# umautobots/LONER

Measured on AMD Instinct MI355X. Metric: training rays/sec, higher is better.
Workload: dtype f32

## Files before the change

### loner_amd/csrc/lnr_density_bf3.hip

```cpp
#include "lnr_f16_common.h"

typedef __bf16 bf16x8 __attribute__((ext_vector_type(8)));
typedef __bf16 bf16x2 __attribute__((ext_vector_type(2)));

#define BF3_TS 36
#ifndef LNR_BF3_FWD_OCC
#define LNR_BF3_FWD_OCC 3
#endif

struct Frag3 { u32x4 t[3]; };

__device__ __forceinline__ void bf3_split_pair(float x, float y, uint32_t& p0, uint32_t& p1, uint32_t& p2) {
    p0 = __builtin_bit_cast(uint32_t, bf16x2{(__bf16)x, (__bf16)y});
    asm volatile("" : "+v"(p0));
    float rx = x - __uint_as_float(p0 << 16), ry = y - __uint_as_float(p0 & 0xFFFF0000u);
    p1 = __builtin_bit_cast(uint32_t, bf16x2{(__bf16)rx, (__bf16)ry});
    asm volatile("" : "+v"(p1));
    rx -= __uint_as_float(p1 << 16);
    ry -= __uint_as_float(p1 & 0xFFFF0000u);
    p2 = __builtin_bit_cast(uint32_t, bf16x2{(__bf16)rx, (__bf16)ry});
}
__device__ __forceinline__ void bf3_split8(const float v[8], Frag3& f) {
#pragma unroll
    for (int q = 0; q < 4; ++q) {
        uint32_t p0, p1, p2;
        bf3_split_pair(v[2 * q], v[2 * q + 1], p0, p1, p2);
        f.t[0][q] = p0; f.t[1][q] = p1; f.t[2][q] = p2;
    }
}
#define BF3_M(a, b, acc) __builtin_amdgcn_mfma_f32_16x16x32_bf16(__builtin_bit_cast(bf16x8, a), __builtin_bit_cast(bf16x8, b), acc, 0, 0, 0)
#define BF3_FOR_TERMS(X) X(0, 2) X(2, 0) X(1, 1) X(0, 1) X(1, 0) X(0, 0)
__device__ __forceinline__ f32x4 bf3_mfma6(const Frag3& a, const Frag3& b, f32x4 acc) {
    acc = BF3_M(a.t[0], b.t[2], acc);
    acc = BF3_M(a.t[2], b.t[0], acc);
    acc = BF3_M(a.t[1], b.t[1], acc);
    acc = BF3_M(a.t[0], b.t[1], acc);
    acc = BF3_M(a.t[1], b.t[0], acc);
    acc = BF3_M(a.t[0], b.t[0], acc);
    return acc;
}

__device__ __forceinline__ void bf3_load_x2(const float* __restrict__ fb, uint32_t plane_bytes, uint32_t m_even, float x[2][8]) {
#pragma unroll
    for (int i = 0; i < 8; ++i) {
        const float2 v = ld32<float2>(fb, (uint32_t)i * plane_bytes + m_even * 4u);
        x[0][i] = v.x; x[1][i] = v.y;
    }
}

template <int HT>
__global__ void __launch_bounds__(LNR_DENSITY_BLOCK, LNR_BF3_FWD_OCC)
mlp_forward_bf3_kernel(const float* __restrict__ params, const float* __restrict__ feat, int64_t m_pad, int64_t n_points,
                       const int32_t* __restrict__ n_rays_dev, int n_rays, int n_samples, float* __restrict__ sigma, int32_t* __restrict__ clip_flag) {
    constexpr int H = 16 * HT;
    const int lane = threadIdx.x & 63, wave = threadIdx.x >> 6, nw = blockDim.x >> 6;
    const int c = lane & 15, g = lane >> 4;
    Frag3 wa[HT]; float wo[HT][4];
#pragma unroll
    for (int jt = 0; jt < HT; ++jt) {
        float v[8];
#pragma unroll
        for (int i = 0; i < 8; ++i) v[i] = params[(16 * jt + c) * 32 + 8 * g + i];
        bf3_split8(v, wa[jt]);
#pragma unroll
        for (int r = 0; r < 4; ++r) wo[jt][r] = params[H * 32 + 16 * jt + 4 * g + r];
    }
    const int64_t M = live_samples(n_points, n_rays_dev, n_rays, n_samples);
    const int64_t n_tiles = M > 0 ? (M + 31) / 32 : 0;
    const int64_t stride = (int64_t)gridDim.x * nw;
    int64_t tile = (int64_t)blockIdx.x * nw + wave;
    if (tile >= n_tiles) return;
    const float* fb = feat + (size_t)(8 * g) * m_pad;
    const uint32_t plane_bytes = (uint32_t)m_pad * 4u;
    float cur[2][8], nxt[2][8];
    bf3_load_x2(fb, plane_bytes, (uint32_t)(tile * 32 + 2 * c), cur);
    bf3_load_x2(fb, plane_bytes, (uint32_t)((tile + stride < n_tiles ? tile + stride : tile) * 32 + 2 * c), nxt);
    while (tile < n_tiles) {
        const int64_t nt = tile + stride, nt2 = nt + stride;
        float nx2[2][8];
        bf3_load_x2(fb, plane_bytes, (uint32_t)((nt2 < n_tiles ? nt2 : tile) * 32 + 2 * c), nx2);
        __builtin_amdgcn_sched_barrier(0);
        Frag3 xb0, xb1;
        bf3_split8(cur[0], xb0);
        bf3_split8(cur[1], xb1);
        f32x4 Z0[HT], Z1[HT];
#pragma unroll
        for (int jt = 0; jt < HT; ++jt) { Z0[jt] = f32x4{0.0f, 0.0f, 0.0f, 0.0f}; Z1[jt] = f32x4{0.0f, 0.0f, 0.0f, 0.0f}; }
#define BF3_X(IA, IB)                                                                          \
    _Pragma("unroll") for (int jt = 0; jt < HT; ++jt) { Z0[jt] = BF3_M(wa[jt].t[IA], xb0.t[IB], Z0[jt]); Z1[jt] = BF3_M(wa[jt].t[IA], xb1.t[IB], Z1[jt]); }
        BF3_FOR_TERMS(BF3_X)
#undef BF3_X
        float p0 = 0.0f, p1 = 0.0f;
#pragma unroll
        for (int jt = 0; jt < HT; ++jt)
#pragma unroll
            for (int r = 0; r < 4; ++r) { p0 += wo[jt][r] * fmaxf(Z0[jt][r], 0.0f); p1 += wo[jt][r] * fmaxf(Z1[jt][r], 0.0f); }
        p0 += __shfl_xor(p0, 16, 64); p1 += __shfl_xor(p1, 16, 64);
        p0 += __shfl_xor(p0, 32, 64); p1 += __shfl_xor(p1, 32, 64);
        const int64_t m = tile * 32 + 2 * c;
        if (g == 0 && m < M) {
            p0 = finite_or_clipped<false>(p0, clip_flag);
            if (m + 1 < M) { p1 = finite_or_clipped<false>(p1, clip_flag); *reinterpret_cast<float2*>(sigma + m) = make_float2(p0, p1); }
            else sigma[m] = p0;
        }
#pragma unroll
        for (int t = 0; t < 2; ++t)
#pragma unroll
            for (int i = 0; i < 8; ++i) { cur[t][i] = nxt[t][i]; nxt[t][i] = nx2[t][i]; }
        tile = nt;
    }
}

template <int HT>
struct Bf3Lds {
    static constexpr int H = 16 * HT, KB = (HT + 1) / 2, NW = LNR_DENSITY_BLOCK / 64;
    static constexpr size_t N_MLP = (size_t)H * 32 + 16 * H;
    static constexpr size_t OFF_T = N_MLP * sizeof(float);
    static constexpr size_t OFF_WA = OFF_T + (size_t)NW * H * BF3_TS * sizeof(float);
    static constexpr size_t OFF_WT = OFF_WA + (size_t)3 * HT * 64 * 16;
    static constexpr size_t BYTES = OFF_WT + (size_t)3 * 2 * KB * 64 * 16;
};

template <int HT>
__global__ void __launch_bounds__(LNR_DENSITY_BLOCK, 2)
mlp_backward_bf3_kernel(const float* __restrict__ params, int n_mlp, const float* __restrict__ feat, int64_t m_pad, int64_t n_points,
                        const int32_t* __restrict__ n_rays_dev, int n_rays, int n_samples, const float* __restrict__ d_sigma,
                        float* __restrict__ dfeat, float* __restrict__ slabs, int want_dfeat) {
    extern __shared__ __attribute__((aligned(16))) float smem[];
    using L = Bf3Lds<HT>;
    constexpr int H = 16 * HT, KB = L::KB;
    const int nw = blockDim.x >> 6;
    const int lane = threadIdx.x & 63, wave = threadIdx.x >> 6;
    const int c = lane & 15, g = lane >> 4;
    float* dW = smem;
    float* T = reinterpret_cast<float*>(reinterpret_cast<char*>(smem) + L::OFF_T) + wave * (H * BF3_TS);
    u32x4* WA = reinterpret_cast<u32x4*>(reinterpret_cast<char*>(smem) + L::OFF_WA);
    u32x4* WT = reinterpret_cast<u32x4*>(reinterpret_cast<char*>(smem) + L::OFF_WT);
    for (int i = threadIdx.x; i < n_mlp; i += blockDim.x) dW[i] = 0.0f;
    for (int job = wave; job < HT + 2 * KB; job += nw) {
        float v[8];
        if (job < HT) {
#pragma unroll
            for (int i = 0; i < 8; ++i) v[i] = params[(16 * job + c) * 32 + 8 * g + i];
        } else {
            const int it = (job - HT) / KB, kb = (job - HT) % KB;
#pragma unroll
            for (int i = 0; i < 8; ++i) {
                const int n = 32 * kb + (i < 4 ? 4 * g + i : 16 + 4 * g + (i - 4));
                v[i] = n < H ? params[n * 32 + 16 * it + c] : 0.0f;
            }
        }
        Frag3 f;
        bf3_split8(v, f);
#pragma unroll
        for (int t3 = 0; t3 < 3; ++t3) {
            if (job < HT) WA[(t3 * HT + job) * 64 + lane] = f.t[t3];
            else WT[(t3 * 2 * KB + (job - HT)) * 64 + lane] = f.t[t3];
        }
    }
    float wo[HT][4];
#pragma unroll
    for (int jt = 0; jt < HT; ++jt)
#pragma unroll
        for (int r = 0; r < 4; ++r) wo[jt][r] = params[H * 32 + 16 * jt + 4 * g + r];
    __syncthreads();
    f32x4 dW1_acc[HT][2];
    float dWo_acc[HT][4];
#pragma unroll
    for (int jt = 0; jt < HT; ++jt) {
        dW1_acc[jt][0] = f32x4{0.0f, 0.0f, 0.0f, 0.0f};
        dW1_acc[jt][1] = f32x4{0.0f, 0.0f, 0.0f, 0.0f};
#pragma unroll
        for (int r = 0; r < 4; ++r) dWo_acc[jt][r] = 0.0f;
    }

    const int64_t M = live_samples(n_points, n_rays_dev, n_rays, n_samples);
    const int64_t n_tiles = M > 0 ? (M + 31) / 32 : 0;
    const int64_t stride = (int64_t)gridDim.x * nw;
    const uint32_t plane_bytes = (uint32_t)m_pad * 4u;
    const float* fb = feat + (size_t)(8 * g) * m_pad;
    const float* fc = feat + (size_t)c * m_pad;
    float* db = dfeat + (size_t)(4 * g) * m_pad;
    int64_t tile = (int64_t)blockIdx.x * nw + wave;
    float xcur[2][8], dcur[2];
    auto load_front = [&](int64_t tl, float (&x)[2][8], float (&ds)[2]) {
        const int64_t m = tl * 32 + 2 * c;
        bf3_load_x2(fb, plane_bytes, (uint32_t)m, x);
        const float v0 = d_sigma[m < M ? m : M - 1], v1 = d_sigma[m + 1 < M ? m + 1 : M - 1];
        ds[0] = m < M ? v0 : 0.0f;
        ds[1] = m + 1 < M ? v1 : 0.0f;
    };
    float xnxt[2][8], dnxt[2];
    if (tile < n_tiles) { load_front(tile, xcur, dcur); load_front(tile + stride < n_tiles ? tile + stride : tile, xnxt, dnxt); }
    while (tile < n_tiles) {
        const int64_t nt = tile + stride;
        const int64_t nt2 = nt + stride;
        float xnx2[2][8], dnx2[2];
        load_front(nt2 < n_tiles ? nt2 : tile, xnx2, dnx2);
        const bool any = (dcur[0] != 0.0f) | (dcur[1] != 0.0f);
        if (__ballot(any) == 0ull) {
            if (want_dfeat) {
#pragma unroll
                for (int k = 0; k < 8; ++k)
                    st32<float2>(db, (uint32_t)(16 * (k >> 2) + (k & 3)) * plane_bytes + (uint32_t)(tile * 32 + 2 * c) * 4u, make_float2(0.0f, 0.0f));
            }
        } else {
            float xraw[2][8];
#pragma unroll
            for (int it = 0; it < 2; ++it) {
                const uint32_t off = (uint32_t)(16 * it) * plane_bytes + (uint32_t)(tile * 32 + 8 * g) * 4u;
                const float4 a = ld32<float4>(fc, off), b = ld32<float4>(fc, off + 16u);
                xraw[it][0] = a.x; xraw[it][1] = a.y; xraw[it][2] = a.z; xraw[it][3] = a.w;
                xraw[it][4] = b.x; xraw[it][5] = b.y; xraw[it][6] = b.z; xraw[it][7] = b.w;
            }
            Frag3 xf[2];
            bf3_split8(xcur[0], xf[0]);
            bf3_split8(xcur[1], xf[1]);
            int wl = lane;
            asm volatile("" : "+v"(wl));
            float dz[HT][2][4];
#pragma unroll
            for (int jt = 0; jt < HT; ++jt) {
                Frag3 wa;
#pragma unroll
                for (int t3 = 0; t3 < 3; ++t3) wa.t[t3] = WA[(t3 * HT + jt) * 64 + wl];
                f32x4 Z0 = f32x4{0.0f, 0.0f, 0.0f, 0.0f}, Z1 = f32x4{0.0f, 0.0f, 0.0f, 0.0f};
#define BF3_X(IA, IB) Z0 = BF3_M(wa.t[IA], xf[0].t[IB], Z0); Z1 = BF3_M(wa.t[IA], xf[1].t[IB], Z1);
                BF3_FOR_TERMS(BF3_X)
#undef BF3_X
#pragma unroll
                for (int r = 0; r < 4; ++r) {
                    dWo_acc[jt][r] += dcur[0] * fmaxf(Z0[r], 0.0f) + dcur[1] * fmaxf(Z1[r], 0.0f);
                    dz[jt][0][r] = Z0[r] > 0.0f ? dcur[0] * wo[jt][r] : 0.0f;
                    dz[jt][1][r] = Z1[r] > 0.0f ? dcur[1] * wo[jt][r] : 0.0f;
                    *reinterpret_cast<float2*>(T + (16 * jt + 4 * g + r) * BF3_TS + 2 * c) = make_float2(dz[jt][0][r], dz[jt][1][r]);
                }
            }
            Frag3 xs[2];
            bf3_split8(xraw[0], xs[0]);
            bf3_split8(xraw[1], xs[1]);
#pragma unroll
            for (int it = 0; it < 2; ++it)
#pragma unroll
                for (int t3 = 0; t3 < 3; ++t3) asm volatile("" : "+v"(xs[it].t[t3]));
            if (want_dfeat) {
                f32x4 D[2][2];
#pragma unroll
                for (int t = 0; t < 2; ++t) {
                    D[t][0] = f32x4{0.0f, 0.0f, 0.0f, 0.0f}; D[t][1] = f32x4{0.0f, 0.0f, 0.0f, 0.0f};
#pragma unroll
                    for (int kb = 0; kb < KB; ++kb) {
                        constexpr bool odd = (HT & 1) != 0;
                        float v[8];
#pragma unroll
                        for (int i = 0; i < 4; ++i) {
                            v[i] = dz[2 * kb][t][i];
                            v[4 + i] = (odd && 2 * kb + 1 >= HT) ? 0.0f : dz[(2 * kb + 1 < HT) ? 2 * kb + 1 : 2 * kb][t][i];
                        }
                        Frag3 b;
                        bf3_split8(v, b);
#pragma unroll
                        for (int it = 0; it < 2; ++it) {
                            Frag3 a;
#pragma unroll
                            for (int t3 = 0; t3 < 3; ++t3) a.t[t3] = WT[((t3 * 2 + it) * KB + kb) * 64 + wl];
                            D[t][it] = bf3_mfma6(a, b, D[t][it]);
                        }
                    }
                }
#pragma unroll
                for (int it = 0; it < 2; ++it)
#pragma unroll
                    for (int r = 0; r < 4; ++r)
                        st32<float2>(db, (uint32_t)(16 * it + r) * plane_bytes + (uint32_t)(tile * 32 + 2 * c) * 4u, make_float2(D[0][it][r], D[1][it][r]));
            }
            __builtin_amdgcn_fence(__ATOMIC_RELEASE, "wavefront");
            __builtin_amdgcn_wave_barrier();
            __builtin_amdgcn_fence(__ATOMIC_ACQUIRE, "wavefront");
#pragma unroll
            for (int jt = 0; jt < HT; ++jt) {
                const float4 a0 = *reinterpret_cast<const float4*>(T + (16 * jt + c) * BF3_TS + 8 * g);
                const float4 a1 = *reinterpret_cast<const float4*>(T + (16 * jt + c) * BF3_TS + 8 * g + 4);
                const float v[8] = {a0.x, a0.y, a0.z, a0.w, a1.x, a1.y, a1.z, a1.w};
                Frag3 a;
                bf3_split8(v, a);
#define BF3_X(IA, IB) dW1_acc[jt][0] = BF3_M(a.t[IA], xs[0].t[IB], dW1_acc[jt][0]); dW1_acc[jt][1] = BF3_M(a.t[IA], xs[1].t[IB], dW1_acc[jt][1]);
                BF3_FOR_TERMS(BF3_X)
#undef BF3_X
            }
            __builtin_amdgcn_fence(__ATOMIC_RELEASE, "wavefront");
            __builtin_amdgcn_wave_barrier();
        }
#pragma unroll
        for (int t = 0; t < 2; ++t) {
#pragma unroll
            for (int i = 0; i < 8; ++i) { xcur[t][i] = xnxt[t][i]; xnxt[t][i] = xnx2[t][i]; }
            dcur[t] = dnxt[t]; dnxt[t] = dnx2[t];
        }
        tile = nt;
    }
    float* dW1 = dW;
    float* dWo = dW + H * 32;
    for (int turn = 0; turn < nw; ++turn) {
        if (wave == turn) {
#pragma unroll
            for (int jt = 0; jt < HT; ++jt) {
#pragma unroll
                for (int it = 0; it < 2; ++it)
#pragma unroll
                    for (int r = 0; r < 4; ++r) dW1[(16 * jt + 4 * g + r) * 32 + 16 * it + c] += dW1_acc[jt][it][r];
#pragma unroll
                for (int r = 0; r < 4; ++r) {
                    float v = dWo_acc[jt][r];
                    v += __shfl_xor(v, 1, 64); v += __shfl_xor(v, 2, 64); v += __shfl_xor(v, 4, 64); v += __shfl_xor(v, 8, 64);
                    if (c == 0) dWo[16 * jt + 4 * g + r] += v;
                }
            }
        }
        __syncthreads();
    }
    float* slab = slabs + (size_t)blockIdx.x * n_mlp;
    for (int i = threadIdx.x; i < n_mlp; i += blockDim.x) slab[i] = dW[i];
}

bool lnr_bf3_class(const LnrNetSpec* spec, int64_t n_points) {
    return spec->precision == LNR_PREC_F32 && spec->encoding == LNR_ENC_HASHGRID && spec->activation == LNR_ACT_RELU && spec->n_hidden == 1 &&
           spec->in_dim == 32 && spec->enc_dim == 32 && spec->n_neurons <= 64 && (spec->n_neurons == 16 || spec->n_neurons == 32 || spec->n_neurons == 64) &&
           n_points <= (1ll << 25) - 2048;
}

int lnr_mlp_fwd_bf3(const MlpArgs& a) {
    const MlpPoints* pt = a.pt;
    const dim3 grid((unsigned)a.route->grid), block(LNR_DENSITY_BLOCK);
#define LNR_BF3_FWD(HT) hipLaunchKernelGGL(mlp_forward_bf3_kernel<HT>, grid, block, 0, a.st, a.params, a.feat, a.m_pad, pt->n_points, pt->n_rays_dev, pt->n_rays, pt->n_samples, a.sigma, pt->clip_flag)
    switch (a.spec->n_neurons / 16) {
        case 1: LNR_BF3_FWD(1); break;
        case 2: LNR_BF3_FWD(2); break;
        default: LNR_BF3_FWD(4); break;
    }
#undef LNR_BF3_FWD
    return LNR_OK;
}

int lnr_mlp_bwd_bf3(const MlpArgs& a) {
    const MlpPoints* pt = a.pt;
    const dim3 grid((unsigned)a.route->grid), block(LNR_DENSITY_BLOCK);
#define LNR_BF3_BWD(HT)                                                                                                          \
    do {                                                                                                                         \
        int rc_ = f16_set_lds(mlp_backward_bf3_kernel<HT>, Bf3Lds<HT>::BYTES, "lnr_density_backward");                           \
        if (rc_) return rc_;                                                                                                     \
        hipLaunchKernelGGL(mlp_backward_bf3_kernel<HT>, grid, block, Bf3Lds<HT>::BYTES, a.st, a.params, a.spec->n_mlp_params, a.feat, a.m_pad, \
                           pt->n_points, pt->n_rays_dev, pt->n_rays, pt->n_samples, a.d_sigma, a.dfeat, a.slabs, a.want_dfeat); \
    } while (0)
    switch (a.spec->n_neurons / 16) {
        case 1: LNR_BF3_BWD(1); break;
        case 2: LNR_BF3_BWD(2); break;
        default: LNR_BF3_BWD(4); break;
    }
#undef LNR_BF3_BWD
    return LNR_OK;
}

__global__ void selftest_mfma_bf3_kernel(float* out) {
    const int lane = threadIdx.x;
    const int c = lane & 15, g = lane >> 4;
    auto A = [](int i, int k) { return (float)((i * 397 + k * 1013) % 4093 - 2046) * 0.015625f; };
    auto B = [](int k, int j) { return (float)((k * 743 - j * 211) % 3571 - 1785) * 0.015625f; };
    float av[8], bv[8];
    for (int i = 0; i < 8; ++i) { av[i] = A(c, 8 * g + i); bv[i] = B(8 * g + i, c); }
    Frag3 a, b;
    bf3_split8(av, a);
    bf3_split8(bv, b);
    const f32x4 d = bf3_mfma6(a, b, f32x4{0.0f, 0.0f, 0.0f, 0.0f});
    float err = 0.0f;
    for (int r = 0; r < 4; ++r) {
        double ref = 0.0;
        for (int k = 0; k < 32; ++k) ref += (double)A(4 * g + r, k) * (double)B(k, c);
        err = fmaxf(err, fabsf((float)(ref - (double)d[r])));
    }
    const float x = 1.0f + (float)(lane * 2654435 % 8388607) * 1.1920929e-7f;
    uint32_t p0, p1, p2;
    bf3_split_pair(x, -x, p0, p1, p2);
    const float back = (__uint_as_float(p0 << 16) + __uint_as_float(p1 << 16)) + __uint_as_float(p2 << 16);
    const float backy = (__uint_as_float(p0 & 0xFFFF0000u) + __uint_as_float(p1 & 0xFFFF0000u)) + __uint_as_float(p2 & 0xFFFF0000u);
    if (back != x || backy != -x) err = 1e9f;
    err = wave_max(err);
    if (lane == 0) out[2] = err;
}

int lnr_selftest_mfma_bf3(float* out, hipStream_t st) {
    hipLaunchKernelGGL(selftest_mfma_bf3_kernel, dim3(1), dim3(64), 0, st, out);
    return LNR_OK;
}
```

Baseline: 2.030 million.

## Transpose features through LDS instead of reloading, rotate prefetch buffers, templatize dfeat

The backward MLP kernel no longer issues a second, column-strided global load of the features for the weight-gradient transpose. It writes the already-prefetched row fragments into the per-wave LDS scratch and reads them back transposed, which needs a larger scratch (TR rows) and extra wave barriers. The triple-buffered prefetch now rotates through three named buffers in a manually unrolled loop instead of copying arrays each iteration. want_dfeat becomes a template parameter, and the wave index is made scalar with readfirstlane.

```diff
diff --git a/loner_amd/csrc/lnr_density_bf3.hip b/loner_amd/csrc/lnr_density_bf3.hip
--- a/loner_amd/csrc/lnr_density_bf3.hip
+++ b/loner_amd/csrc/lnr_density_bf3.hip
@@ -113,27 +113,27 @@
 
 template <int HT>
 struct Bf3Lds {
-    static constexpr int H = 16 * HT, KB = (HT + 1) / 2, NW = LNR_DENSITY_BLOCK / 64;
+    static constexpr int H = 16 * HT, KB = (HT + 1) / 2, NW = LNR_DENSITY_BLOCK / 64, TR = H < 32 ? 32 : H;
     static constexpr size_t N_MLP = (size_t)H * 32 + 16 * H;
     static constexpr size_t OFF_T = N_MLP * sizeof(float);
-    static constexpr size_t OFF_WA = OFF_T + (size_t)NW * H * BF3_TS * sizeof(float);
+    static constexpr size_t OFF_WA = OFF_T + (size_t)NW * TR * BF3_TS * sizeof(float);
     static constexpr size_t OFF_WT = OFF_WA + (size_t)3 * HT * 64 * 16;
     static constexpr size_t BYTES = OFF_WT + (size_t)3 * 2 * KB * 64 * 16;
 };
 
-template <int HT>
+template <int HT, bool WANT_DFEAT>
 __global__ void __launch_bounds__(LNR_DENSITY_BLOCK, 2)
 mlp_backward_bf3_kernel(const float* __restrict__ params, int n_mlp, const float* __restrict__ feat, int64_t m_pad, int64_t n_points,
                         const int32_t* __restrict__ n_rays_dev, int n_rays, int n_samples, const float* __restrict__ d_sigma,
-                        float* __restrict__ dfeat, float* __restrict__ slabs, int want_dfeat) {
+                        float* __restrict__ dfeat, float* __restrict__ slabs) {
     extern __shared__ __attribute__((aligned(16))) float smem[];
     using L = Bf3Lds<HT>;
     constexpr int H = 16 * HT, KB = L::KB;
     const int nw = blockDim.x >> 6;
-    const int lane = threadIdx.x & 63, wave = threadIdx.x >> 6;
+    const int lane = threadIdx.x & 63, wave = __builtin_amdgcn_readfirstlane((int)(threadIdx.x >> 6));
     const int c = lane & 15, g = lane >> 4;
     float* dW = smem;
-    float* T = reinterpret_cast<float*>(reinterpret_cast<char*>(smem) + L::OFF_T) + wave * (H * BF3_TS);
+    float* T = reinterpret_cast<float*>(reinterpret_cast<char*>(smem) + L::OFF_T) + wave * (L::TR * BF3_TS);
     u32x4* WA = reinterpret_cast<u32x4*>(reinterpret_cast<char*>(smem) + L::OFF_WA);
     u32x4* WT = reinterpret_cast<u32x4*>(reinterpret_cast<char*>(smem) + L::OFF_WT);
     for (int i = threadIdx.x; i < n_mlp; i += blockDim.x) dW[i] = 0.0f;
@@ -179,40 +179,33 @@
     const int64_t stride = (int64_t)gridDim.x * nw;
     const uint32_t plane_bytes = (uint32_t)m_pad * 4u;
     const float* fb = feat + (size_t)(8 * g) * m_pad;
-    const float* fc = feat + (size_t)c * m_pad;
     float* db = dfeat + (size_t)(4 * g) * m_pad;
     int64_t tile = (int64_t)blockIdx.x * nw + wave;
-    float xcur[2][8], dcur[2];
+    const int64_t tile0 = tile;
     auto load_front = [&](int64_t tl, float (&x)[2][8], float (&ds)[2]) {
         const int64_t m = tl * 32 + 2 * c;
         bf3_load_x2(fb, plane_bytes, (uint32_t)m, x);
-        const float v0 = d_sigma[m < M ? m : M - 1], v1 = d_sigma[m + 1 < M ? m + 1 : M - 1];
-        ds[0] = m < M ? v0 : 0.0f;
-        ds[1] = m + 1 < M ? v1 : 0.0f;
+        ds[0] = d_sigma[m < M ? m : M - 1];
+        ds[1] = d_sigma[m + 1 < M ? m + 1 : M - 1];
     };
-    float xnxt[2][8], dnxt[2];
-    if (tile < n_tiles) { load_front(tile, xcur, dcur); load_front(tile + stride < n_tiles ? tile + stride : tile, xnxt, dnxt); }
-    while (tile < n_tiles) {
-        const int64_t nt = tile + stride;
+    auto step = [&](const float (&xcur)[2][8], const float (&draw)[2], float (&xpre)[2][8], float (&dpre)[2]) {
+        const int64_t nt = tile + stride, m0 = tile * 32 + 2 * c;
+        const float dcur[2] = {m0 < M ? draw[0] : 0.0f, m0 + 1 < M ? draw[1] : 0.0f};
         const int64_t nt2 = nt + stride;
-        float xnx2[2][8], dnx2[2];
-        load_front(nt2 < n_tiles ? nt2 : tile, xnx2, dnx2);
+        load_front(nt2 < n_tiles ? nt2 : tile0, xpre, dpre);
+        if (tile >= n_tiles) { tile = nt; return; }
+        const uint32_t st_off = (uint32_t)(tile * 32 + 2 * c) * 4u;
         const bool any = (dcur[0] != 0.0f) | (dcur[1] != 0.0f);
         if (__ballot(any) == 0ull) {
-            if (want_dfeat) {
+            if (WANT_DFEAT) {
 #pragma unroll
                 for (int k = 0; k < 8; ++k)
-                    st32<float2>(db, (uint32_t)(16 * (k >> 2) + (k & 3)) * plane_bytes + (uint32_t)(tile * 32 + 2 * c) * 4u, make_float2(0.0f, 0.0f));
+                    st32<float2>(db, (uint32_t)(16 * (k >> 2) + (k & 3)) * plane_bytes + st_off, make_float2(0.0f, 0.0f));
             }
         } else {
-            float xraw[2][8];
-#pragma unroll
-            for (int it = 0; it < 2; ++it) {
-                const uint32_t off = (uint32_t)(16 * it) * plane_bytes + (uint32_t)(tile * 32 + 8 * g) * 4u;
-                const float4 a = ld32<float4>(fc, off), b = ld32<float4>(fc, off + 16u);
-                xraw[it][0] = a.x; xraw[it][1] = a.y; xraw[it][2] = a.z; xraw[it][3] = a.w;
-                xraw[it][4] = b.x; xraw[it][5] = b.y; xraw[it][6] = b.z; xraw[it][7] = b.w;
-            }
+#pragma unroll
+            for (int i = 0; i < 8; ++i)
+                *reinterpret_cast<float2*>(T + (8 * g + i) * BF3_TS + 2 * c) = make_float2(xcur[0][i], xcur[1][i]);
             Frag3 xf[2];
             bf3_split8(xcur[0], xf[0]);
             bf3_split8(xcur[1], xf[1]);
@@ -230,20 +223,35 @@
 #undef BF3_X
 #pragma unroll
                 for (int r = 0; r < 4; ++r) {
-                    dWo_acc[jt][r] += dcur[0] * fmaxf(Z0[r], 0.0f) + dcur[1] * fmaxf(Z1[r], 0.0f);
+                    const float a0 = fmaxf(Z0[r], 0.0f), a1 = fmaxf(Z1[r], 0.0f);
+                    dWo_acc[jt][r] += (r & 1) ? __builtin_fmaf(dcur[1], a1, dcur[0] * a0) : __builtin_fmaf(dcur[0], a0, dcur[1] * a1);
                     dz[jt][0][r] = Z0[r] > 0.0f ? dcur[0] * wo[jt][r] : 0.0f;
                     dz[jt][1][r] = Z1[r] > 0.0f ? dcur[1] * wo[jt][r] : 0.0f;
+                }
+            }
+            __builtin_amdgcn_fence(__ATOMIC_RELEASE, "wavefront");
+            __builtin_amdgcn_wave_barrier();
+            __builtin_amdgcn_fence(__ATOMIC_ACQUIRE, "wavefront");
+            Frag3 xs[2];
+#pragma unroll
+            for (int it = 0; it < 2; ++it) {
+                const float4 a = *reinterpret_cast<const float4*>(T + (16 * it + c) * BF3_TS + 8 * g);
+                const float4 b = *reinterpret_cast<const float4*>(T + (16 * it + c) * BF3_TS + 8 * g + 4);
+                const float xraw[8] = {a.x, a.y, a.z, a.w, b.x, b.y, b.z, b.w};
+                bf3_split8(xraw, xs[it]);
+            }
+            __builtin_amdgcn_fence(__ATOMIC_RELEASE, "wavefront");
+            __builtin_amdgcn_wave_barrier();
+#pragma unroll
+            for (int jt = 0; jt < HT; ++jt)
+#pragma unroll
+                for (int r = 0; r < 4; ++r)
                     *reinterpret_cast<float2*>(T + (16 * jt + 4 * g + r) * BF3_TS + 2 * c) = make_float2(dz[jt][0][r], dz[jt][1][r]);
-                }
-            }
-            Frag3 xs[2];
-            bf3_split8(xraw[0], xs[0]);
-            bf3_split8(xraw[1], xs[1]);
 #pragma unroll
             for (int it = 0; it < 2; ++it)
 #pragma unroll
                 for (int t3 = 0; t3 < 3; ++t3) asm volatile("" : "+v"(xs[it].t[t3]));
-            if (want_dfeat) {
+            if (WANT_DFEAT) {
                 f32x4 D[2][2];
 #pragma unroll
                 for (int t = 0; t < 2; ++t) {
@@ -272,7 +280,7 @@
                 for (int it = 0; it < 2; ++it)
 #pragma unroll
                     for (int r = 0; r < 4; ++r)
-                        st32<float2>(db, (uint32_t)(16 * it + r) * plane_bytes + (uint32_t)(tile * 32 + 2 * c) * 4u, make_float2(D[0][it][r], D[1][it][r]));
+                        st32<float2>(db, (uint32_t)(16 * it + r) * plane_bytes + st_off, make_float2(D[0][it][r], D[1][it][r]));
             }
             __builtin_amdgcn_fence(__ATOMIC_RELEASE, "wavefront");
             __builtin_amdgcn_wave_barrier();
@@ -291,13 +299,15 @@
             __builtin_amdgcn_fence(__ATOMIC_RELEASE, "wavefront");
             __builtin_amdgcn_wave_barrier();
         }
-#pragma unroll
-        for (int t = 0; t < 2; ++t) {
-#pragma unroll
-            for (int i = 0; i < 8; ++i) { xcur[t][i] = xnxt[t][i]; xnxt[t][i] = xnx2[t][i]; }
-            dcur[t] = dnxt[t]; dnxt[t] = dnx2[t];
-        }
         tile = nt;
+    };
+    float xa[2][8], xb[2][8], xc[2][8], da[2], dbb[2], dc[2];
+    if (tile < n_tiles) { load_front(tile, xa, da); load_front(tile + stride < n_tiles ? tile + stride : tile, xb, dbb); }
+    __builtin_amdgcn_s_waitcnt(0x0F70);
+    while (tile < n_tiles) {
+        step(xa, da, xc, dc);
+        step(xb, dbb, xa, da);
+        step(xc, dc, xb, dbb);
     }
     float* dW1 = dW;
     float* dWo = dW + H * 32;
@@ -345,18 +355,20 @@
 int lnr_mlp_bwd_bf3(const MlpArgs& a) {
     const MlpPoints* pt = a.pt;
     const dim3 grid((unsigned)a.route->grid), block(LNR_DENSITY_BLOCK);
-#define LNR_BF3_BWD(HT)                                                                                                          \
+#define LNR_BF3_BWD_(HT, DF)                                                                                                     \
     do {                                                                                                                         \
-        int rc_ = f16_set_lds(mlp_backward_bf3_kernel<HT>, Bf3Lds<HT>::BYTES, "lnr_density_backward");                           \
+        int rc_ = f16_set_lds(mlp_backward_bf3_kernel<HT, DF>, Bf3Lds<HT>::BYTES, "lnr_density_backward");                       \
         if (rc_) return rc_;                                                                                                     \
-        hipLaunchKernelGGL(mlp_backward_bf3_kernel<HT>, grid, block, Bf3Lds<HT>::BYTES, a.st, a.params, a.spec->n_mlp_params, a.feat, a.m_pad, \
-                           pt->n_points, pt->n_rays_dev, pt->n_rays, pt->n_samples, a.d_sigma, a.dfeat, a.slabs, a.want_dfeat); \
+        hipLaunchKernelGGL((mlp_backward_bf3_kernel<HT, DF>), grid, block, Bf3Lds<HT>::BYTES, a.st, a.params, a.spec->n_mlp_params, a.feat, a.m_pad, \
+                           pt->n_points, pt->n_rays_dev, pt->n_rays, pt->n_samples, a.d_sigma, a.dfeat, a.slabs);                \
     } while (0)
+#define LNR_BF3_BWD(HT) do { if (a.want_dfeat) LNR_BF3_BWD_(HT, true); else LNR_BF3_BWD_(HT, false); } while (0)
     switch (a.spec->n_neurons / 16) {
         case 1: LNR_BF3_BWD(1); break;
         case 2: LNR_BF3_BWD(2); break;
         default: LNR_BF3_BWD(4); break;
     }
+#undef LNR_BF3_BWD_
 #undef LNR_BF3_BWD
     return LNR_OK;
 }
```

Result: faster. 2.053 million, median of 6 (+1.1%).
